# ablab/stringdecomposer

Measured on NVIDIA B200. Metric: dp_gcups, higher is better.
Workload: dtype s16x2

## Files before the change

stringdecomposer_b200/csrc/sweep_kernels.cu:

```cuda
#include <cuda_runtime.h>
#include <nvtx3/nvToolsExt.h>

#include <algorithm>
#include <climits>
#include <cstdio>
#include <cstdlib>
#include <cstring>
#include <mutex>
#include <string>
#include <vector>

#include "sweep_kernel.cuh"
#include "sweep_lat_kernel.cuh"
#include "filter_kernels.cuh"
#include "cuda_scope.h"
#include "block_cache.h"

namespace sdb {

#define SD_CUDA(x)                                                                                              \
    do {                                                                                                        \
        cudaError_t e_ = (x);                                                                                   \
        if (e_ != cudaSuccess) throw PlanError{std::string("CUDA error: ") + cudaGetErrorString(e_) + " at " +  \
                                               __FILE__ + ":" + std::to_string(__LINE__)};                      \
    } while (0)

struct TbArgs {
    Geometry g;
    const uint32_t *codes; const int64_t *cta_code_off;
    const JR *jr; const int64_t *seg_j_off;
    const uint8_t *bases; const int64_t *seg_off; int nseg;
    const uint8_t *rows; const int *row_off;
    int ins, del, mismatch, match;
    Record *scratch; const int64_t *seg_rec_off; int *counts;
    const int *rank2row;
    int *error;
    int invC;
};

constexpr int TB_WARPS = 4;
__global__ void __launch_bounds__(TB_WARPS * 32) traceback_kernel(const TbArgs a)
{
    const int s = blockIdx.x * TB_WARPS + (threadIdx.x >> 5);
    if (s >= a.nseg) return;
    const int lane = threadIdx.x & 31;
    const Geometry g = a.g;
    const int cta0 = g.NG > 1 ? s * g.NG : s / g.NS, seg_local = g.NG > 1 ? 0 : s % g.NS;
    const int64_t o = a.seg_off[s];
    const int n = (int)(a.seg_off[s + 1] - o);
    const uint8_t *seg = a.bases + o;
    const JR *jr = a.jr + a.seg_j_off[s];
    const size_t cstride = (size_t)g.NT * g.CW;
    const int C = g.C, CW = g.CW, cshift = g.packed ? 3 : 4, cpw = 1 << cshift, invC = a.invC;
    const int maxwl = g.T * CW - 1;
    Record *out = a.scratch + a.seg_rec_off[s];

    const int *r2r = a.rank2row ? a.rank2row + (size_t)s * (2 * g.M) : nullptr;
    auto row_of = [&](int kr) { return (unsigned)kr >= (unsigned)(2 * g.M) ? -1 : r2r ? r2r[kr] : kr; };
    int i = n - 1;
    int r = row_of(jr[n].row);
    if (r < 0) {
        if (lane == 0) { *a.error = 1; a.counts[s] = 0; }
        return;
    }
    int last = a.row_off[r + 1] - a.row_off[r] - 1;
    int k = last, end = i, end_score = jr[n].j, cnt = 0;
    constexpr int TB_RING = 8;
    __shared__ uint32_t s_ring[TB_WARPS][TB_RING][4][32];
    uint32_t (*ring)[4][32] = s_ring[threadIdx.x >> 5];
    int i0 = -1000, row0 = -1, half = 0, ni0 = -2000, cur = 0;
    uint32_t w0 = 0, w1 = 0, w2 = 0; int wb = 0; bool colok = false;
    const uint32_t *rowbase = nullptr;
    auto issue_window = [&](int slot, int iw, int kw) {
        const int c = iw - lane;
        const bool xok = c >= 0 && kw >= 1;
        int xb = 0;
        if (xok) {
            const int kp = max(kw - lane, 0);
            const int t = (kp * invC) >> 16;
            const int wl = t * CW + ((kp - t * C) >> cshift);
            xb = min(max(wl - 1, 0), max(maxwl - 2, 0));
            const uint32_t *col = rowbase + (size_t)c * cstride;
            const uint32_t d0 = (uint32_t)__cvta_generic_to_shared(&ring[slot][0][lane]);
            asm volatile("cp.async.ca.shared.global [%0], [%1], 4;" ::"r"(d0), "l"(col + xb) : "memory");
            asm volatile("cp.async.ca.shared.global [%0], [%1], 4;" ::"r"(d0 + 128u), "l"(col + min(xb + 1, maxwl)) : "memory");
            asm volatile("cp.async.ca.shared.global [%0], [%1], 4;" ::"r"(d0 + 256u), "l"(col + min(xb + 2, maxwl)) : "memory");
        }
        ring[slot][3][lane] = (uint32_t)xb | (xok ? 0x80000000u : 0u);
        asm volatile("cp.async.commit_group;" ::: "memory");
    };

    for (;;) {
        if (k == 0) {
            bool ins_move = false;
            if (i != 0) {
                const uint8_t m0 = a.rows[a.row_off[r]];
                const int s_here = m0 == seg[i] ? a.match : a.mismatch;
                const int s_prev = m0 == seg[i - 1] ? a.match : a.mismatch;
                const int h_here = jr[i].j + s_here;
                const int h_prev = (i == 1) ? s_prev : jr[i - 1].j + s_prev;
                ins_move = (h_here == h_prev + a.ins);
            }
            if (ins_move) { --i; continue; }
        } else {
            if (r != row0 || i > i0 || i <= i0 - 32) {
                if (r == row0 && i == ni0) {
                    i0 = ni0;
                    const int freed = cur;
                    cur = cur + 1 == TB_RING ? 0 : cur + 1;
                    issue_window(freed, i0 - 32 * (TB_RING - 1), k - 32 * (TB_RING - 1));
                } else {
                    i0 = i; row0 = r;
                    const RowPlace pl = place_row(g, seg_local, r);
                    half = pl.half;
                    rowbase = a.codes + a.cta_code_off[cta0 + (g.NG > 1 ? pl.grp : 0)] + (size_t)lane_tid(g.T, pl.ginst, 0) * CW;
                    asm volatile("cp.async.wait_all;" ::: "memory");
                    cur = 0;
#pragma unroll
                    for (int j = 0; j < TB_RING; ++j) issue_window(j, i - 32 * j, k - 32 * j);
                }
                ni0 = i0 - 32;
                asm volatile("cp.async.wait_group %0;" ::"n"(TB_RING - 1) : "memory");
                w0 = ring[cur][0][lane]; w1 = ring[cur][1][lane]; w2 = ring[cur][2][lane];
                const uint32_t meta = ring[cur][3][lane];
                wb = (int)(meta & 0x7fffffffu); colok = (meta >> 31) != 0;
            }
            const int dcur = i0 - i;
            const int kd = k - (lane - dcur);
            bool ok = colok && lane >= dcur && kd >= 1;
            int code = 2;
            {
                const int kq = max(kd, 0);
                const int t = (kq * invC) >> 16;
                const int kk = kq - t * C;
                const int wi = kk >> cshift;
                const int rel = t * CW + wi - wb;
                ok = ok && (unsigned)rel < 3u;
                const uint32_t w = rel == 0 ? w0 : rel == 1 ? w1 : w2;
                const int cc = kk & (cpw - 1);
                const int ncell = min(cpw, C - (wi << cshift));
                code = decode_code(w, g.packed, ncell, cc, half);
            }
            const bool stop = lane >= dcur && (!ok || code != 2);
            const unsigned ball = __ballot_sync(0xffffffffu, stop);
            const int f = ball ? __ffs(ball) - 1 : 32;
            const int steps = f - dcur;
            i -= steps; k -= steps;
            if (f == 32) continue;
            const int okf = __shfl_sync(0xffffffffu, (int)ok, f);
            const int codef = __shfl_sync(0xffffffffu, code, f);
            if (!okf) {
                if (k >= 1) row0 = -1;
                continue;
            }
            if (codef == 0) { --k; continue; }
            if (codef == 1) { --i; continue; }
        }
        if (cnt >= n) { cnt = -1; break; }
        Record rec;
        rec.row = r; rec.start = i; rec.end = end;
        if (i == 0) { rec.score = end_score; if (lane == 0) out[cnt] = rec; ++cnt; break; }
        const JR ji = jr[i];
        rec.score = end_score - ji.j;
        if (lane == 0) out[cnt] = rec;
        ++cnt;
        end_score = ji.j;
        r = row_of(ji.row);
        if (r < 0) {
            if (lane == 0) *a.error = 1;
            cnt = 0;
            break;
        }
        --i;
        last = a.row_off[r + 1] - a.row_off[r] - 1;
        k = last; end = i;
    }
    if (lane == 0) a.counts[s] = cnt;
}

__global__ void __launch_bounds__(1024) gather_kernel(const Record *scratch, const int64_t *seg_rec_off, const int *counts, Record *dense,
                                                      int nseg, int *total)
{
    __shared__ int s_warp[32];
    __shared__ int s_base, s_bad;
    const int tid = threadIdx.x, lane = tid & 31, warp = tid >> 5;
    if (tid == 0) { s_base = 0; s_bad = 0; }
    __syncthreads();
    for (int c0 = 0; c0 < nseg; c0 += 1024) {
        const int s = c0 + tid;
        const int c = s < nseg ? counts[s] : 0;
        if (c < 0) s_bad = 1;
        int v = c < 0 ? 0 : c;
#pragma unroll
        for (int d = 1; d < 32; d <<= 1) { const int o = __shfl_up_sync(0xffffffffu, v, d); if (lane >= d) v += o; }
        if (lane == 31) s_warp[warp] = v;
        __syncthreads();
        if (warp == 0) {
            int w = s_warp[lane];
#pragma unroll
            for (int d = 1; d < 32; d <<= 1) { const int o = __shfl_up_sync(0xffffffffu, w, d); if (lane >= d) w += o; }
            s_warp[lane] = w;
        }
        __syncthreads();
        const int start = s_base + (warp ? s_warp[warp - 1] : 0) + v - (c < 0 ? 0 : c);
        if (s < nseg && c > 0) {
            const Record *src = scratch + seg_rec_off[s];
            Record *dst = dense + start;
            for (int x = 0; x < c; ++x) dst[x] = src[c - 1 - x];
        }
        __syncthreads();
        if (tid == 0) s_base += s_warp[31];
        __syncthreads();
    }
    if (tid == 0) *total = s_bad ? -1 : s_base;
}

template <int MODE> __global__ void int_peak_kernel(unsigned *out, unsigned seed)
{
    unsigned r[8];
    const unsigned b = seed * 3u + threadIdx.x;
#pragma unroll
    for (int j = 0; j < 8; ++j) r[j] = threadIdx.x * 17u + j * 1315423911u + seed;
    for (int it = 0; it < 2048; ++it) {
#pragma unroll
        for (int j = 0; j < 8; ++j) {
            const unsigned nb = r[(j + 1) & 7];
            if (MODE == 0) r[j] = __viaddmax_s16x2(r[j], b, nb);
            else { r[j] = __viaddmax_s16x2(r[j], b, nb); r[j] = r[j] * b + nb; }
        }
    }
    unsigned acc = 0;
#pragma unroll
    for (int j = 0; j < 8; ++j) acc ^= r[j];
    out[blockIdx.x * blockDim.x + threadIdx.x] = acc;
}

static const void *sweep_kernel_for(const Geometry &g, bool fast, bool multi, bool timing)
{
    static const SweepLookup classic[2][3][2] = {
        {{sweep_lookup_s32_f0_m0, sweep_lookup_s32_f0_m0_st}, {sweep_lookup_s32_f1_m0, sweep_lookup_s32_f1_m0_st},
         {sweep_lookup_s32_f1_m1, sweep_lookup_s32_f1_m1_st}},
        {{sweep_lookup_p16_f0_m0, sweep_lookup_p16_f0_m0_st}, {sweep_lookup_p16_f1_m0, sweep_lookup_p16_f1_m0_st},
         {sweep_lookup_p16_f1_m1, sweep_lookup_p16_f1_m1_st}}};
    static const SweepLookup group[2] = {sweep_group_lookup_s32, sweep_group_lookup_p16};
    static const SweepLookup lat[2][2] = {{sweep_lat_lookup_s32, sweep_lat_lookup_s32_st}, {sweep_lat_lookup_p16, sweep_lat_lookup_p16_st}};
    const int pol = g.packed ? 1 : 0, st = g.stream ? 1 : 0;
    if (g.lat && timing) return pol && !st ? sweep_lat_timing_lookup_p16(g) : nullptr;
    if (g.lat) return lat[pol][st](g);
    if (g.NG > 1) return group[pol](g);
    return classic[pol][fast ? (multi ? 2 : 1) : 0][st](g);
}

namespace {

struct DevBuf {
    void *p = nullptr; size_t cap = 0; int dev = -1;
    void release()
    {
        if (!p) return;
// ... 57 lines not shown
constexpr size_t OUT_HDR = 16;
inline size_t out_counts_bytes(int nseg) { return ((size_t)nseg * 4 + 15) & ~size_t(15); }
inline int64_t wave_total(const int *hdr)
{
    if (hdr[1]) throw PlanError{"CUDA: sweep timed out waiting for a partner CTA (internal error)"};
    if (hdr[3]) throw PlanError{SD_MSG_TB_BAD_ROW};
    if (hdr[0]) throw PlanError{"segment contains a symbol outside ACGTN"};
    if (hdr[2] < 0) throw PlanError{"traceback overflowed its record buffer (internal error)"};
    return hdr[2];
}

struct WaveSlot {
    DevBuf d_bases, d_meta, d_codes, d_jr, d_scratch, d_out, d_dist, d_rank, d_r2r, d_segkj, d_xchg, d_dbg;
    MetaView d_segoff, d_ctanmax, d_ctacode, d_segj, d_segrec;
    PinnedBuf h_out;
    std::vector<char> hmeta;
    std::vector<int64_t> hoff;
    CtaLayout lay;
    int s0 = 0, s1 = 0, nseg = 0, nmax = 0;
    bool filter_on = false, staged = false;
    size_t nb = 0, rec_guess = 0;
    int end_idx = -1, prev_end = -1;
    cudaEvent_t ev[7]{};
};

class CudaBackend : public Backend {
public:
    explicit CudaBackend(int dev) : dev_(dev)
    {
        DeviceScope scope_(dev_); SD_CUDA(scope_.status);
        SD_CUDA(cudaStreamCreateWithFlags(&st_, cudaStreamNonBlocking));
        SD_CUDA(cudaStreamCreateWithFlags(&st_in_, cudaStreamNonBlocking));
        SD_CUDA(cudaStreamCreateWithFlags(&st_out_, cudaStreamNonBlocking));
        SD_CUDA(cudaStreamCreateWithFlags(&st_tb_, cudaStreamNonBlocking));
        SD_CUDA(cudaStreamCreateWithFlags(&st2_, cudaStreamNonBlocking));
        for (auto &w : slot_) for (auto &e : w.ev) SD_CUDA(cudaEventCreate(&e));
        for (auto &e : endev_) SD_CUDA(cudaEventCreate(&e));
        SD_CUDA(cudaGetDeviceProperties(&prop_, dev_));
        if (prop_.major != 10) throw PlanError{"CUDA device is not sm_100 class: this library carries sm_100a code only (no PTX for other architectures)"};
        size_t fr = 0, tot = 0;
        SD_CUDA(cudaMemGetInfo(&fr, &tot));
        free_at_start_ = (int64_t)fr;
        budget_ = std::min<int64_t>((int64_t)(fr * 0.85), (int64_t)96 << 30);
    }
    ~CudaBackend() override
    {
        DeviceScope scope_(dev_);
        cudaDeviceSynchronize();
        for (auto &w : slot_) for (auto &e : w.ev) cudaEventDestroy(e);
        for (auto &e : endev_) cudaEventDestroy(e);
        cudaStreamDestroy(st2_);
        cudaStreamDestroy(st_); cudaStreamDestroy(st_in_); cudaStreamDestroy(st_out_); cudaStreamDestroy(st_tb_);
    }
    const char *name() const override { return "cuda"; }

    void configure(const Plan &p, const MonomerSet &ms) override
    {
        DeviceScope scope_(dev_); SD_CUDA(scope_.status);
        plan_ = p; ms_ = ms;
        const Geometry &g = p.g;
        const int spw = 32 / g.T;
        fast_ = (g.nslots % spw == 0) && (g.nslots / spw <= 4) && g.NS <= 15;
        if (getenv("SD_NOFAST")) fast_ = false;
        lat_timing_ = g.lat && getenv("SD_LAT_TIMING") && sweep_kernel_for(g, fast_, false, true);
        kernel_ = sweep_kernel_for(g, fast_, fast_ && g.NS > 1, lat_timing_);
        if (g.lat && (g.NT / 32) * g.NG > 32) throw PlanError{"internal: a deferred-jump cluster holds at most 32 warps"};
        if (!kernel_) throw PlanError{"no sweep kernel compiled for this geometry"};
        cudaFuncAttributes fa;
        SD_CUDA(cudaFuncGetAttributes(&fa, kernel_));
        const int nthreads = g.NT * (g.NG > 1 && !g.lat ? g.NS : 1);
        if ((int64_t)((fa.numRegs + 7) / 8 * 8) * nthreads > 65536 || fa.maxThreadsPerBlock < nthreads)
            throw PlanError{"sweep geometry exceeds the register file (regs*threads > 64K)"};
        const std::vector<uint32_t> &table = g.lat ? p.prof2 : p.prof;
        d_prof_.need(table.size() * 4);
        SD_CUDA(cudaMemcpyAsync(d_prof_.p, table.data(), table.size() * 4, cudaMemcpyHostToDevice, st_));
        d_slotlen_.need(p.slot_len.size() * 4); d_slotend_.need(p.slot_endadd.size() * 4);
        SD_CUDA(cudaMemcpyAsync(d_slotlen_.p, p.slot_len.data(), p.slot_len.size() * 4, cudaMemcpyHostToDevice, st_));
        SD_CUDA(cudaMemcpyAsync(d_slotend_.p, p.slot_endadd.data(), p.slot_endadd.size() * 4, cudaMemcpyHostToDevice, st_));
        d_rows_.need(ms.rows.size()); d_rowoff_.need(ms.row_off.size() * 4);
        rows_ascii_.resize(ms.rows.size());
        for (size_t x = 0; x < ms.rows.size(); ++x) rows_ascii_[x] = (uint8_t)"ACGTN"[ms.rows[x]];
        SD_CUDA(cudaMemcpyAsync(d_rows_.p, rows_ascii_.data(), rows_ascii_.size(), cudaMemcpyHostToDevice, st_));
        SD_CUDA(cudaMemcpyAsync(d_rowoff_.p, ms.row_off.data(), ms.row_off.size() * 4, cudaMemcpyHostToDevice, st_));
        if (g.lat) {
            const int R = ms.nrows();
            kjbase_.assign((size_t)R * 5, 0);
            std::vector<int> one((size_t)R, -1);
            for (int r = 0; r < R; ++r) {
                one[(size_t)r] = 0;
                lat_jump_keys(ms, p.sc, one.data(), kjbase_.data() + (size_t)r * 5);
                one[(size_t)r] = -1;
            }
            d_kjbase_.need(kjbase_.size() * 4);
            SD_CUDA(cudaMemcpyAsync(d_kjbase_.p, kjbase_.data(), kjbase_.size() * 4, cudaMemcpyHostToDevice, st_));
        }
        SD_CUDA(cudaStreamSynchronize(st_));
    }

    int64_t wave_bytes(const Batch &b, int s0, int s1) const override
    {
        CtaLayout l = make_cta_layout(plan_, b, s0, s1);
        int64_t bytes = l.cta_code_off.back() * 4 + l.seg_j_off.back() * 8 + l.seg_rec_off.back() * 32 + (b.off[s1] - b.off[s0]);
        if (ed_thr_ >= 0) bytes += (int64_t)(s1 - s0) * ms_.nrows() * 12;
        return bytes;
    }
    int64_t wave_budget() const override
    {
        if (const char *e = getenv("SD_WAVE_BYTES")) if (atoll(e) > 0) return atoll(e);
        return budget_;
    }
    int64_t device_bytes() const override { return free_at_start_; }
    int wave_slots() const override { return 2; }

    void reserve(int slot, const Batch &b, int s0, int s1) override
    {
        DeviceScope scope_(dev_); SD_CUDA(scope_.status);
        WaveSlot &w = slot_[slot & 1];
        const CtaLayout lay = make_cta_layout(plan_, b, s0, s1);
        const int nseg = s1 - s0;
        w.d_bases.need((size_t)(b.off[s1] - b.off[s0]) + 16);
        w.d_codes.need((size_t)lay.cta_code_off.back() * 4 + 16);
        w.d_jr.need((size_t)lay.seg_j_off.back() * sizeof(JR) + 16);
        w.d_scratch.need((size_t)lay.seg_rec_off.back() * sizeof(Record) + 16);
        w.d_out.need(OUT_HDR + out_counts_bytes(nseg) + (size_t)lay.seg_rec_off.back() * sizeof(Record) + 64);
        w.h_out.need(OUT_HDR + out_counts_bytes(nseg) + ((size_t)(b.off[s1] - b.off[s0]) / 48 + (size_t)nseg * 4 + 64) * sizeof(Record));
    }

    void enqueue_h2d(WaveSlot &w, const Batch &b, int s0, int s1)
    {
        w.s0 = s0; w.s1 = s1; w.nseg = s1 - s0;
        w.lay = make_cta_layout(plan_, b, s0, s1);
        w.nmax = 0;
        for (int v : w.lay.cta_nmax) w.nmax = std::max(w.nmax, v);
        const int64_t base = b.off[s0];
        w.nb = (size_t)(b.off[s1] - base);
        w.hoff.resize((size_t)w.nseg + 1);
        for (int s = 0; s <= w.nseg; ++s) w.hoff[s] = b.off[s0 + s] - base;
        w.d_bases.need(w.nb + 16);
        const size_t msz[5] = {w.hoff.size() * 8, w.lay.cta_nmax.size() * 4, w.lay.cta_code_off.size() * 8, w.lay.seg_j_off.size() * 8,
                               w.lay.seg_rec_off.size() * 8};
        const void *msrc[5] = {w.hoff.data(), w.lay.cta_nmax.data(), w.lay.cta_code_off.data(), w.lay.seg_j_off.data(), w.lay.seg_rec_off.data()};
        MetaView *mdst[5] = {&w.d_segoff, &w.d_ctanmax, &w.d_ctacode, &w.d_segj, &w.d_segrec};
        size_t mtotal = 0, moff[5];
        for (int x = 0; x < 5; ++x) { moff[x] = mtotal; mtotal += (msz[x] + 255) & ~size_t(255); }
        w.d_meta.need(mtotal + 16);
        w.hmeta.resize(mtotal);
        for (int x = 0; x < 5; ++x) { memcpy(w.hmeta.data() + moff[x], msrc[x], msz[x]); mdst[x]->p = w.d_meta.as<char>() + moff[x]; }
        w.d_codes.need((size_t)w.lay.cta_code_off.back() * 4 + 16);
        w.d_jr.need((size_t)w.lay.seg_j_off.back() * sizeof(JR) + 16);
        w.d_scratch.need((size_t)w.lay.seg_rec_off.back() * sizeof(Record) + 16);
        w.rec_guess = (size_t)(w.nb / 48) + (size_t)w.nseg * 4 + 64;
        w.d_out.need(OUT_HDR + out_counts_bytes(w.nseg) + (size_t)w.lay.seg_rec_off.back() * sizeof(Record) + 64);
        SD_CUDA(cudaEventRecord(w.ev[0], st_in_));
        SD_CUDA(cudaMemcpyAsync(w.d_bases.p, b.text + base, w.nb, cudaMemcpyHostToDevice, st_in_));
        SD_CUDA(cudaMemcpyAsync(w.d_meta.p, w.hmeta.data(), mtotal, cudaMemcpyHostToDevice, st_in_));
        SD_CUDA(cudaMemsetAsync(w.d_out.p, 0, OUT_HDR, st_in_));
        SD_CUDA(cudaEventRecord(w.ev[1], st_in_));
        h2d_bytes += (int64_t)(w.nb + mtotal);
        w.filter_on = ed_thr_ >= 0;
        if (w.filter_on) build_filter(w);
        w.staged = true;
    }

    void build_filter(WaveSlot &w)
    {
        const int R = ms_.nrows();
        const size_t np = (size_t)w.nseg * R;
        w.d_dist.need(np * 4); w.d_rank.need(np * 4); w.d_r2r.need(np * 4);
        int *segkj = nullptr;
        if (plan_.g.lat) { w.d_segkj.need((size_t)w.nseg * 5 * 4); segkj = w.d_segkj.as<int>(); }
        SD_CUDA(launch_filter(w.d_bases.as<uint8_t>(), w.d_segoff.as<int64_t>(), w.nseg, w.nmax, d_rows_.as<uint8_t>(), d_rowoff_.as<int>(),
// ... 49 lines not shown
        a.error = w.d_out.as<int>() + 1;
        const int spw = 32 / g.T, wps = g.NT / 32;
        const size_t sgt = (size_t)wps * spw * g.T;
        const size_t smem = (size_t)5 * sgt * plan_.qp * 16 + ((size_t)g.NS * wps + g.NS + 8) * 4;
        if (smem > (size_t)prop_.sharedMemPerBlockOptin) throw PlanError{"group sweep needs more shared memory than the SM has"};
        SD_CUDA(cudaFuncSetAttribute(kernel_, cudaFuncAttributeMaxDynamicSharedMemorySize, (int)smem));
        int per_sm = 0;
        SD_CUDA(cudaOccupancyMaxActiveBlocksPerMultiprocessor(&per_sm, kernel_, g.NS * g.NT, smem));
        const int capacity = per_sm * prop_.multiProcessorCount;
        if (capacity < g.NG) throw PlanError{"monomer set too large: the CTAs of one segment cannot be co-resident on this GPU"};
        const int nblocks = (w.nseg + g.NS - 1) / g.NS;
        a.ngslots = std::min(nblocks, capacity / g.NG);
        if (const char *e = getenv("SD_GROUP_GSLOTS")) if (atoi(e) > 0) a.ngslots = std::min(a.ngslots, atoi(e));
        group_slots = std::max(group_slots, a.ngslots);
        const size_t xwords = (size_t)a.ngslots * 2 * g.NG * g.NS;
        w.d_xchg.need(xwords * 8);
        a.xbuf = w.d_xchg.as<unsigned long long>();
        SD_CUDA(cudaMemsetAsync(a.xbuf, 0, xwords * 8, st_));
        void *args[] = {(void *)&a};
        SD_CUDA(cudaLaunchCooperativeKernel(kernel_, dim3(a.ngslots * g.NG), dim3(g.NS * g.NT), args, smem, st_));
    }

    void launch_lat(WaveSlot &w, int seg_stride)
    {
        const Geometry &g = plan_.g;
        LatArgs a;
        fill_common_args(a, w);
        a.prof2 = d_prof_.as<uint4>(); a.nsl_total = plan_.nsl; a.qp2 = plan_.qp2;
        a.NG = g.NG; a.SG = g.SG;
        a.lat_th = plan_.lat_th; a.scanw = g.scanw;
        for (int q = 0; q < 5; ++q) a.kj[q] = plan_.kj[q];
        a.seg_kj = w.filter_on ? w.d_segkj.as<int>() : nullptr;
        a.seg_stride = seg_stride;
        a.error = w.d_out.as<int>() + 1;
        const int spw = 32 / g.T, wpc = g.NT / 32;
        a.dbg = nullptr;
        if (lat_timing_) { w.d_dbg.need((size_t)w.nseg * g.NG * wpc * 64); a.dbg = w.d_dbg.as<long long>(); SD_CUDA(cudaMemsetAsync(a.dbg, 0, (size_t)w.nseg * g.NG * wpc * 64, st_)); }
        const size_t sgt = (size_t)wpc * spw * g.T;
        const size_t smem = (size_t)5 * sgt * plan_.qp2 * 16 + (size_t)LAT_NBUF * 32 * 8 + 32 + (g.stream ? 0 : (size_t)seg_stride);
        if (smem > (size_t)prop_.sharedMemPerBlockOptin) throw PlanError{"deferred-jump sweep needs more shared memory than the SM has"};
        SD_CUDA(cudaFuncSetAttribute(kernel_, cudaFuncAttributeMaxDynamicSharedMemorySize, (int)smem));
        cudaLaunchConfig_t cfg{};
        cfg.gridDim = dim3((unsigned)(w.nseg * g.NG)); cfg.blockDim = dim3((unsigned)g.NT);
        cfg.dynamicSmemBytes = smem; cfg.stream = st_;
        cudaLaunchAttribute attr[1];
        attr[0].id = cudaLaunchAttributeClusterDimension;
        attr[0].val.clusterDim.x = (unsigned)g.NG; attr[0].val.clusterDim.y = 1; attr[0].val.clusterDim.z = 1;
        cfg.attrs = attr; cfg.numAttrs = 1;
        void *args[] = {(void *)&a};
        SD_CUDA(cudaLaunchKernelExC(&cfg, kernel_, args));
        if (lat_timing_) {
            const size_t nw = (size_t)w.nseg * g.NG * wpc;
            std::vector<long long> h(nw * 8);
            SD_CUDA(cudaMemcpyAsync(h.data(), a.dbg, nw * 64, cudaMemcpyDeviceToHost, st_));
            SD_CUDA(cudaStreamSynchronize(st_));
            double acc[6] = {0, 0, 0, 0, 0, 0}, cols = 0;
            for (size_t x = 0; x < nw; ++x) { for (int q = 0; q < 6; ++q) acc[q] += (double)h[x * 8 + q]; cols += (double)h[x * 8 + 6]; }
            fprintf(stderr, "[sd_b200 lat timing] cycles per column and warp: scan %.1f chain %.1f key+publish %.1f receive %.1f J+merge+store %.1f pre %.1f  (total %.1f)\n",
                    acc[0] / cols, acc[1] / cols, acc[2] / cols, acc[3] / cols, acc[4] / cols, acc[5] / cols,
                    (acc[0] + acc[1] + acc[2] + acc[3] + acc[4] + acc[5]) / cols);
        }
    }

    void enqueue_kernels(WaveSlot &w)
    {
        const Geometry &g = plan_.g;
        const int seg_stride = (w.nmax + 16) / 16 * 16;
        const bool own_stream = !g.lat && g.NG == 1 && &w == &slot_[1];
        cudaStream_t ss = own_stream ? st2_ : st_;
        SD_CUDA(cudaStreamWaitEvent(ss, w.ev[1], 0));
        SD_CUDA(cudaEventRecord(w.ev[2], ss));
        if (g.lat) launch_lat(w, seg_stride); else if (g.NG > 1) launch_group(w); else launch_single(w, seg_stride, ss);
        SD_CUDA(cudaEventRecord(w.ev[3], ss));
        w.prev_end = last_end_;
        w.end_idx = (int)(wave_seq_++ & 3);
        SD_CUDA(cudaEventRecord(endev_[w.end_idx], ss));
        last_end_ = w.end_idx;
        SD_CUDA(cudaStreamWaitEvent(st_tb_, w.ev[3], 0));
        SD_CUDA(cudaEventRecord(w.ev[6], st_tb_));
        TbArgs t;
        t.g = g; t.codes = w.d_codes.as<uint32_t>(); t.cta_code_off = w.d_ctacode.as<int64_t>(); t.jr = w.d_jr.as<JR>();
        t.seg_j_off = w.d_segj.as<int64_t>();
        t.bases = w.d_bases.as<uint8_t>(); t.seg_off = w.d_segoff.as<int64_t>(); t.nseg = w.nseg;
        t.rows = d_rows_.as<uint8_t>(); t.row_off = d_rowoff_.as<int>();
        t.ins = plan_.sc.ins; t.del = plan_.sc.del; t.mismatch = plan_.sc.mismatch; t.match = plan_.sc.match;
        t.scratch = w.d_scratch.as<Record>(); t.seg_rec_off = w.d_segrec.as<int64_t>();
        t.counts = reinterpret_cast<int *>(w.d_out.as<char>() + OUT_HDR);
        t.rank2row = w.filter_on ? w.d_r2r.as<int>() : nullptr;
        t.error = w.d_out.as<int>() + 3;
        t.invC = (65536 + g.C - 1) / g.C;
        for (int pos = 0; pos < g.C * g.T; ++pos)
            if (((pos * t.invC) >> 16) != pos / g.C) throw PlanError{"internal: reciprocal division inexact"};
        traceback_kernel<<<(w.nseg + TB_WARPS - 1) / TB_WARPS, TB_WARPS * 32, 0, st_tb_>>>(t);
        SD_CUDA(cudaGetLastError());
        SD_CUDA(cudaEventRecord(w.ev[4], st_tb_));
        launches += 2;
    }

    void enqueue_gather(WaveSlot &w)
    {
        char *ob = w.d_out.as<char>();
        Record *dense = reinterpret_cast<Record *>(ob + OUT_HDR + out_counts_bytes(w.nseg));
        gather_kernel<<<1, 1024, 0, st_tb_>>>(w.d_scratch.as<Record>(), w.d_segrec.as<int64_t>(), reinterpret_cast<int *>(ob + OUT_HDR),
                                          dense, w.nseg, reinterpret_cast<int *>(ob) + 2);
        SD_CUDA(cudaGetLastError());
        launches += 1;
    }

    void enqueue_d2h(WaveSlot &w)
    {
        const size_t first = OUT_HDR + out_counts_bytes(w.nseg) + w.rec_guess * sizeof(Record);
        const size_t cap = OUT_HDR + out_counts_bytes(w.nseg) + (size_t)w.lay.seg_rec_off.back() * sizeof(Record);
        w.h_out.need(std::min(first, cap));
        SD_CUDA(cudaEventRecord(w.ev[5], st_tb_));
        SD_CUDA(cudaStreamWaitEvent(st_out_, w.ev[5], 0));
        SD_CUDA(cudaMemcpyAsync(w.h_out.p, w.d_out.p, std::min(first, cap), cudaMemcpyDeviceToHost, st_out_));
        SD_CUDA(cudaEventRecord(w.ev[5], st_out_));
    }

    void finish(WaveSlot &w, BatchResult &out)
    {
        SD_CUDA(cudaEventSynchronize(w.ev[5]));
        const int64_t total = wave_total(w.h_out.as<int>());
        const size_t rec_off = OUT_HDR + out_counts_bytes(w.nseg);
        const size_t base = out.recs.size();
        out.recs.resize(base + (size_t)total);
        const size_t have = std::min<size_t>((size_t)total, w.rec_guess);
        if (have) memcpy(out.recs.data() + base, w.h_out.as<char>() + rec_off, have * sizeof(Record));
        if ((size_t)total > have) {
            SD_CUDA(cudaMemcpyAsync(out.recs.data() + base + have, w.d_out.as<char>() + rec_off + have * sizeof(Record),
                                    ((size_t)total - have) * sizeof(Record), cudaMemcpyDeviceToHost, st_out_));
            SD_CUDA(cudaStreamSynchronize(st_out_));
        }
        const int *cnt = reinterpret_cast<const int *>(w.h_out.as<char>() + OUT_HDR);
        int64_t run = (int64_t)base;
        for (int s = 0; s < w.nseg; ++s) { run += cnt[s]; out.rec_off.push_back(run); }
        float ms = 0;
        SD_CUDA(cudaEventElapsedTime(&ms, w.ev[0], w.ev[1])); h2d_ms += ms;
        SD_CUDA(cudaEventElapsedTime(&ms, w.ev[2], w.ev[3]));
        if (w.prev_end >= 0) {
            float since_prev = 0;
            SD_CUDA(cudaEventElapsedTime(&since_prev, endev_[w.prev_end], w.ev[3]));
            ms = std::min(ms, std::max(since_prev, 0.0f));
        }
        sweep_ms += ms;
        SD_CUDA(cudaEventElapsedTime(&ms, w.ev[6], w.ev[4])); traceback_ms += ms;
        d2h_bytes += (int64_t)(rec_off + (size_t)total * sizeof(Record));
        w.staged = false;
    }

    void submit(int slot, const Batch &b, int s0, int s1) override
    {
        DeviceScope scope_(dev_); SD_CUDA(scope_.status);
        WaveSlot &w = slot_[slot & 1];
        nvtxRangePushA("sd_b200: wave copy-in");
        enqueue_h2d(w, b, s0, s1);
        nvtxRangePop();
        nvtxRangePushA("sd_b200: wave sweep + traceback");
        enqueue_kernels(w);
        enqueue_gather(w);
        nvtxRangePop();
        nvtxRangePushA("sd_b200: wave copy-out");
        enqueue_d2h(w);
        nvtxRangePop();
    }
    void collect(int slot, BatchResult &out) override
    {
        DeviceScope scope_(dev_); SD_CUDA(scope_.status);
        nvtxRangePushA("sd_b200: wave collect");
        try { finish(slot_[slot & 1], out); } catch (...) { nvtxRangePop(); throw; }
        nvtxRangePop();
    }
    void stage(const Batch &b, int s0, int s1) override
    {
        DeviceScope scope_(dev_); SD_CUDA(scope_.status);
        enqueue_h2d(slot_[0], b, s0, s1);
        SD_CUDA(cudaStreamSynchronize(st_in_));
        float ms = 0; SD_CUDA(cudaEventElapsedTime(&ms, slot_[0].ev[0], slot_[0].ev[1])); h2d_ms += ms;
    }
    void execute() override
    {
        DeviceScope scope_(dev_); SD_CUDA(scope_.status);
        WaveSlot &w = slot_[0];
        SD_CUDA(cudaMemsetAsync(w.d_out.p, 0, OUT_HDR, st_));
        enqueue_kernels(w);
        int hdr[4] = {0, 0, 0, 0};
        SD_CUDA(cudaMemcpyAsync(hdr, w.d_out.p, OUT_HDR, cudaMemcpyDeviceToHost, st_tb_));
        SD_CUDA(cudaStreamSynchronize(st_tb_));
        wave_total(hdr);
        float ms = 0;
        SD_CUDA(cudaEventElapsedTime(&ms, w.ev[2], w.ev[3])); sweep_ms += ms;
        SD_CUDA(cudaEventElapsedTime(&ms, w.ev[6], w.ev[4])); traceback_ms += ms;
    }
    void fetch(BatchResult &out) override
    {
        DeviceScope scope_(dev_); SD_CUDA(scope_.status);
        WaveSlot &w = slot_[0];
        const double sw = sweep_ms, tb = traceback_ms, h2 = h2d_ms;
        enqueue_gather(w);
        enqueue_d2h(w);
        finish(w, out);
        sweep_ms = sw; traceback_ms = tb; h2d_ms = h2;
    }

private:
    int dev_;
    cudaStream_t st_{}, st_in_{}, st_out_{}, st_tb_{};
    cudaStream_t st2_{};
    cudaEvent_t endev_[4]{};
    uint64_t wave_seq_ = 0; int last_end_ = -1;
    cudaDeviceProp prop_{};
    Plan plan_; MonomerSet ms_;
    const void *kernel_ = nullptr;
    bool fast_ = false, lat_timing_ = false;
    std::vector<uint8_t> rows_ascii_;
    int64_t budget_ = 0;
    int64_t free_at_start_ = 0;
    DevBuf d_prof_, d_slotlen_, d_slotend_, d_rows_, d_rowoff_, d_kjbase_;
    std::vector<int> kjbase_;
    WaveSlot slot_[2];
};

}

Backend *make_cuda_backend(int device_id, std::string &err)
{
    try { return new CudaBackend(device_id); }
    catch (PlanError &e) { err = e.msg; return nullptr; }
}

}

int cuda_device_count()
{
    int n = 0;
    if (cudaGetDeviceCount(&n) != cudaSuccess) return 0;
    return n;
}

void *cuda_host_alloc(size_t bytes)
{
    void *p = nullptr;
    if (cudaHostAlloc(&p, bytes ? bytes : 1, cudaHostAllocPortable) != cudaSuccess) { cudaGetLastError(); return nullptr; }
    return p;
}

void cuda_host_free(void *p) { cudaFreeHost(p); }

int cuda_int_peak(int device, double *alu, double *both, double *mhz, std::string &err)
{
    using namespace sdb;
    try {
        DeviceScope scope_(device); SD_CUDA(scope_.status);
        cudaDeviceProp p; SD_CUDA(cudaGetDeviceProperties(&p, device));
        const int nblk = p.multiProcessorCount * 2, nthr = 512;
        unsigned *d; SD_CUDA(cudaMalloc(&d, (size_t)nblk * nthr * 4));
        cudaEvent_t e0, e1; SD_CUDA(cudaEventCreate(&e0)); SD_CUDA(cudaEventCreate(&e1));
        double res[2] = {0, 0};
        for (int mode = 0; mode < 2; ++mode) {
            float best = 1e30f;
            for (int rep = 0; rep < 5; ++rep) {
                SD_CUDA(cudaEventRecord(e0));
                if (mode == 0) int_peak_kernel<0><<<nblk, nthr>>>(d, 1234u); else int_peak_kernel<1><<<nblk, nthr>>>(d, 1234u);
                SD_CUDA(cudaEventRecord(e1));
                SD_CUDA(cudaEventSynchronize(e1));
                float ms; SD_CUDA(cudaEventElapsedTime(&ms, e0, e1));
                if (rep > 0) best = std::min(best, ms);
            }
            const double ops = (double)nblk * nthr * 2048.0 * 8.0 * (mode == 0 ? 1.0 : 2.0);
            res[mode] = ops / (best * 1e-3);
        }
        if (alu) *alu = res[0];
        if (both) *both = res[1];
        if (mhz) *mhz = res[0] / ((double)p.multiProcessorCount * 64.0) / 1e6;
        cudaEventDestroy(e0); cudaEventDestroy(e1); cudaFree(d);
    } catch (PlanError &e) { err = e.msg; return 4; }
    return 0;
}
```

Baseline: 2740.

## Prefetch next row's traceback windows and nearby JR/base data into double-buffered shared ring

The traceback kernel now precomputes a per-slot row table (last column, code word offset, group, first symbol, half) on the host, which replaces the place_row, row_off and cta_code_off lookups done inside the kernel. At each row transition it predicts the next row from the JR entry and issues cp.async prefetches of that row's code windows, plus a window of nearby JR records and sequence bytes, into a second shared-memory buffer. Boundary and insertion checks read JR and bases from shared memory through warp shuffles instead of global loads. This aims to hide the global-load latency of the serial traceback chain, at the cost of doubling shared memory per warp and adding more complex wait-group bookkeeping. The codes base now uses cta_code_off[cta0] plus grp*n*cstride, which assumes a particular layout when NG>1.

New measurement: 2697, median of 6. 1.6% lower.

```diff
diff --git a/stringdecomposer_b200/csrc/sweep_kernels.cu b/stringdecomposer_b200/csrc/sweep_kernels.cu
--- a/stringdecomposer_b200/csrc/sweep_kernels.cu
+++ b/stringdecomposer_b200/csrc/sweep_kernels.cu
@@ -25,12 +25,20 @@
                                                __FILE__ + ":" + std::to_string(__LINE__)};                      \
     } while (0)
 
+struct alignas(16) TbRow {
+    int32_t last;
+    int32_t word;
+    int32_t grp;
+    uint8_t sym, half;
+    uint8_t pad_[2];
+};
+
 struct TbArgs {
     Geometry g;
     const uint32_t *codes; const int64_t *cta_code_off;
     const JR *jr; const int64_t *seg_j_off;
     const uint8_t *bases; const int64_t *seg_off; int nseg;
-    const uint8_t *rows; const int *row_off;
+    const TbRow *rowtab;
     int ins, del, mismatch, match;
     Record *scratch; const int64_t *seg_rec_off; int *counts;
     const int *rank2row;
@@ -39,9 +47,13 @@
 };
 
 constexpr int TB_WARPS = 4;
+constexpr int TB_RING = 8;
+constexpr int TB_NEAR = 32;
+constexpr int TB_AIM = 8;
 __global__ void __launch_bounds__(TB_WARPS * 32) traceback_kernel(const TbArgs a)
 {
-    const int s = blockIdx.x * TB_WARPS + (threadIdx.x >> 5);
+    const int wid = threadIdx.x >> 5;
+    const int s = blockIdx.x * TB_WARPS + wid;
     if (s >= a.nseg) return;
     const int lane = threadIdx.x & 31;
     const Geometry g = a.g;
@@ -54,6 +66,13 @@
     const int C = g.C, CW = g.CW, cshift = g.packed ? 3 : 4, cpw = 1 << cshift, invC = a.invC;
     const int maxwl = g.T * CW - 1;
     Record *out = a.scratch + a.seg_rec_off[s];
+    const uint32_t *codes = a.codes + a.cta_code_off[cta0];
+    const TbRow *rowtab = a.rowtab + (size_t)seg_local * (2 * g.M);
+    struct RowInfo { int last, sym, half; const uint32_t *base; };
+    auto row_info = [&](int r) {
+        const uint4 v = __ldg(reinterpret_cast<const uint4 *>(rowtab + r));
+        return RowInfo{(int)v.x, (int)(v.w & 0xffu), (int)((v.w >> 8) & 0xffu), codes + (size_t)v.z * n * cstride + v.y};
+    };
 
     const int *r2r = a.rank2row ? a.rank2row + (size_t)s * (2 * g.M) : nullptr;
     auto row_of = [&](int kr) { return (unsigned)kr >= (unsigned)(2 * g.M) ? -1 : r2r ? r2r[kr] : kr; };
@@ -63,15 +82,18 @@
         if (lane == 0) { *a.error = 1; a.counts[s] = 0; }
         return;
     }
-    int last = a.row_off[r + 1] - a.row_off[r] - 1;
-    int k = last, end = i, end_score = jr[n].j, cnt = 0;
-    constexpr int TB_RING = 8;
-    __shared__ uint32_t s_ring[TB_WARPS][TB_RING][4][32];
-    uint32_t (*ring)[4][32] = s_ring[threadIdx.x >> 5];
-    int i0 = -1000, row0 = -1, half = 0, ni0 = -2000, cur = 0;
+    RowInfo ri = row_info(r);
+    int k = ri.last, end = i, end_score = jr[n].j, cnt = 0;
+    __shared__ uint32_t s_ring[TB_WARPS][2][TB_RING][4][32];
+    __shared__ uint2 s_njr[TB_WARPS][2][TB_NEAR];
+    __shared__ uint32_t s_nsym[TB_WARPS][2][TB_NEAR];
+    int rb = 0, nb = 0;
+    int i0 = -1000, row0 = -1, ni0 = -2000, cur = 0;
     uint32_t w0 = 0, w1 = 0, w2 = 0; int wb = 0; bool colok = false;
-    const uint32_t *rowbase = nullptr;
-    auto issue_window = [&](int slot, int iw, int kw) {
+    int nlo = INT_MIN / 2, nal = 0;
+    int nx_row = -1, nx_i0 = 0, nx_lo = 0, nx_al = 0; RowInfo nx_ri{0, 0, 0, nullptr};
+    int older = 0;
+    auto issue_window = [&](int ringi, const uint32_t *rowbase, int slot, int iw, int kw) {
         const int c = iw - lane;
         const bool xok = c >= 0 && kw >= 1;
         int xb = 0;
@@ -81,49 +103,97 @@
             const int wl = t * CW + ((kp - t * C) >> cshift);
             xb = min(max(wl - 1, 0), max(maxwl - 2, 0));
             const uint32_t *col = rowbase + (size_t)c * cstride;
-            const uint32_t d0 = (uint32_t)__cvta_generic_to_shared(&ring[slot][0][lane]);
+            const uint32_t d0 = (uint32_t)__cvta_generic_to_shared(&s_ring[wid][ringi][slot][0][lane]);
             asm volatile("cp.async.ca.shared.global [%0], [%1], 4;" ::"r"(d0), "l"(col + xb) : "memory");
             asm volatile("cp.async.ca.shared.global [%0], [%1], 4;" ::"r"(d0 + 128u), "l"(col + min(xb + 1, maxwl)) : "memory");
             asm volatile("cp.async.ca.shared.global [%0], [%1], 4;" ::"r"(d0 + 256u), "l"(col + min(xb + 2, maxwl)) : "memory");
         }
-        ring[slot][3][lane] = (uint32_t)xb | (xok ? 0x80000000u : 0u);
+        s_ring[wid][ringi][slot][3][lane] = (uint32_t)xb | (xok ? 0x80000000u : 0u);
         asm volatile("cp.async.commit_group;" ::: "memory");
+    };
+    auto issue_near = [&](int b, int c, int &al) {
+        const int lo = max(0, min(c - TB_NEAR / 2, n + 1 - TB_NEAR));
+        if (lo + lane <= n) {
+            const uint32_t d = (uint32_t)__cvta_generic_to_shared(&s_njr[wid][b][lane]);
+            asm volatile("cp.async.ca.shared.global [%0], [%1], 8;" ::"r"(d), "l"(jr + lo + lane) : "memory");
+        }
+        al = (int)((uintptr_t)(seg + lo) & 3u);
+        const uint8_t *wsrc = seg + lo - al + 4 * lane;
+        if (lane < (TB_NEAR + 3) / 4 + 1 && wsrc < seg + n) {
+            const uint32_t d = (uint32_t)__cvta_generic_to_shared(&s_nsym[wid][b][lane]);
+            asm volatile("cp.async.ca.shared.global [%0], [%1], 4;" ::"r"(d), "l"(wsrc) : "memory");
+        }
+        asm volatile("cp.async.commit_group;" ::: "memory");
+        return lo;
+    };
+    auto close_data = [&](int c, JR &jc, int &jprev, int &sc, int &sprev) {
+        if (c - 1 >= nlo && c < nlo + TB_NEAR) {
+            const uint2 mj = s_njr[wid][nb][lane];
+            const uint32_t ms = s_nsym[wid][nb][lane];
+            jc.j = (int)__shfl_sync(0xffffffffu, mj.x, c - nlo); jc.row = (int)__shfl_sync(0xffffffffu, mj.y, c - nlo);
+            jprev = (int)__shfl_sync(0xffffffffu, mj.x, c - 1 - nlo);
+            const int q = c - nlo + nal;
+            sc = (int)((__shfl_sync(0xffffffffu, ms, q >> 2) >> (8 * (q & 3))) & 0xffu);
+            sprev = (int)((__shfl_sync(0xffffffffu, ms, (q - 1) >> 2) >> (8 * ((q - 1) & 3))) & 0xffu);
+        } else {
+            jc = jr[c]; jprev = jr[c - 1].j; sc = seg[c]; sprev = seg[c - 1];
+        }
+    };
+    auto issue_next = [&]() {
+        const int c = i - k;
+        if (c < 1 || c < nlo || c >= nlo + TB_NEAR) return;
+        const int kr = (int)__shfl_sync(0xffffffffu, s_njr[wid][nb][lane].y, c - nlo);
+        const int nr = row_of(kr);
+        if (nr < 0) return;
+        nx_ri = row_info(nr);
+        const int aim = min(TB_AIM, n - c);
+        nx_row = nr; nx_i0 = c - 1 + aim;
+        nx_lo = issue_near(nb ^ 1, c - 1 - nx_ri.last, nx_al);
+#pragma unroll
+        for (int j = 0; j < TB_RING; ++j) issue_window(rb ^ 1, nx_ri.base, j, nx_i0 - 32 * j, nx_ri.last + aim - 32 * j);
+        older = TB_RING - 1;
     };
 
     for (;;) {
         if (k == 0) {
             bool ins_move = false;
             if (i != 0) {
-                const uint8_t m0 = a.rows[a.row_off[r]];
-                const int s_here = m0 == seg[i] ? a.match : a.mismatch;
-                const int s_prev = m0 == seg[i - 1] ? a.match : a.mismatch;
-                const int h_here = jr[i].j + s_here;
-                const int h_prev = (i == 1) ? s_prev : jr[i - 1].j + s_prev;
+                JR jh; int jp, sh, sp;
+                close_data(i, jh, jp, sh, sp);
+                const int s_here = ri.sym == sh ? a.match : a.mismatch;
+                const int s_prev = ri.sym == sp ? a.match : a.mismatch;
+                const int h_here = jh.j + s_here;
+                const int h_prev = (i == 1) ? s_prev : jp + s_prev;
                 ins_move = (h_here == h_prev + a.ins);
             }
             if (ins_move) { --i; continue; }
         } else {
             if (r != row0 || i > i0 || i <= i0 - 32) {
-                if (r == row0 && i == ni0) {
+                bool fresh = true;
+                if (r == nx_row && i <= nx_i0 && i > nx_i0 - 32) {
+                    asm volatile("cp.async.wait_all;" ::: "memory");
+                    rb ^= 1; nb ^= 1; nlo = nx_lo; nal = nx_al;
+                    i0 = nx_i0; row0 = r; cur = 0; older = 0;
+                } else if (r == row0 && i == ni0) {
                     i0 = ni0;
                     const int freed = cur;
                     cur = cur + 1 == TB_RING ? 0 : cur + 1;
-                    issue_window(freed, i0 - 32 * (TB_RING - 1), k - 32 * (TB_RING - 1));
+                    issue_window(rb, ri.base, freed, i0 - 32 * (TB_RING - 1), k - 32 * (TB_RING - 1));
+                    fresh = false;
                 } else {
-                    i0 = i; row0 = r;
-                    const RowPlace pl = place_row(g, seg_local, r);
-                    half = pl.half;
-                    rowbase = a.codes + a.cta_code_off[cta0 + (g.NG > 1 ? pl.grp : 0)] + (size_t)lane_tid(g.T, pl.ginst, 0) * CW;
                     asm volatile("cp.async.wait_all;" ::: "memory");
-                    cur = 0;
+                    i0 = i; row0 = r; cur = 0; older = 0;
+                    nlo = issue_near(nb, i - k, nal);
 #pragma unroll
-                    for (int j = 0; j < TB_RING; ++j) issue_window(j, i - 32 * j, k - 32 * j);
+                    for (int j = 0; j < TB_RING; ++j) issue_window(rb, ri.base, j, i - 32 * j, k - 32 * j);
                 }
                 ni0 = i0 - 32;
-                asm volatile("cp.async.wait_group %0;" ::"n"(TB_RING - 1) : "memory");
-                w0 = ring[cur][0][lane]; w1 = ring[cur][1][lane]; w2 = ring[cur][2][lane];
-                const uint32_t meta = ring[cur][3][lane];
+                if (older > 0) { --older; asm volatile("cp.async.wait_group %0;" ::"n"(TB_RING - 1 + TB_RING + 1) : "memory"); }
+                else asm volatile("cp.async.wait_group %0;" ::"n"(TB_RING - 1) : "memory");
+                w0 = s_ring[wid][rb][cur][0][lane]; w1 = s_ring[wid][rb][cur][1][lane]; w2 = s_ring[wid][rb][cur][2][lane];
+                const uint32_t meta = s_ring[wid][rb][cur][3][lane];
                 wb = (int)(meta & 0x7fffffffu); colok = (meta >> 31) != 0;
+                if (fresh) { nx_row = -1; issue_next(); }
             }
             const int dcur = i0 - i;
             const int kd = k - (lane - dcur);
@@ -139,7 +209,7 @@
                 const uint32_t w = rel == 0 ? w0 : rel == 1 ? w1 : w2;
                 const int cc = kk & (cpw - 1);
                 const int ncell = min(cpw, C - (wi << cshift));
-                code = decode_code(w, g.packed, ncell, cc, half);
+                code = decode_code(w, g.packed, ncell, cc, ri.half);
             }
             const bool stop = lane >= dcur && (!ok || code != 2);
             const unsigned ball = __ballot_sync(0xffffffffu, stop);
@@ -150,7 +220,7 @@
             const int okf = __shfl_sync(0xffffffffu, (int)ok, f);
             const int codef = __shfl_sync(0xffffffffu, code, f);
             if (!okf) {
-                if (k >= 1) row0 = -1;
+                if (k >= 1) { row0 = -1; nx_row = -1; }
                 continue;
             }
             if (codef == 0) { --k; continue; }
@@ -160,7 +230,8 @@
         Record rec;
         rec.row = r; rec.start = i; rec.end = end;
         if (i == 0) { rec.score = end_score; if (lane == 0) out[cnt] = rec; ++cnt; break; }
-        const JR ji = jr[i];
+        JR ji; int jp_, sh_, sp_;
+        close_data(i, ji, jp_, sh_, sp_);
         rec.score = end_score - ji.j;
         if (lane == 0) out[cnt] = rec;
         ++cnt;
@@ -172,8 +243,8 @@
             break;
         }
         --i;
-        last = a.row_off[r + 1] - a.row_off[r] - 1;
-        k = last; end = i;
+        ri = r == nx_row ? nx_ri : row_info(r);
+        k = ri.last; end = i;
     }
     if (lane == 0) a.counts[s] = cnt;
 }
@@ -398,11 +469,22 @@
         for (size_t x = 0; x < ms.rows.size(); ++x) rows_ascii_[x] = (uint8_t)"ACGTN"[ms.rows[x]];
         SD_CUDA(cudaMemcpyAsync(d_rows_.p, rows_ascii_.data(), rows_ascii_.size(), cudaMemcpyHostToDevice, st_));
         SD_CUDA(cudaMemcpyAsync(d_rowoff_.p, ms.row_off.data(), ms.row_off.size() * 4, cudaMemcpyHostToDevice, st_));
+        const int npos = g.NG > 1 ? 1 : g.NS, nrows = ms.nrows();
+        tbrow_.assign((size_t)npos * nrows, TbRow{});
+        for (int sl = 0; sl < npos; ++sl)
+            for (int r = 0; r < nrows; ++r) {
+                const RowPlace pl = place_row(g, sl, r);
+                TbRow &e = tbrow_[(size_t)sl * nrows + r];
+                e.last = ms.rowlen(r) - 1; e.word = lane_tid(g.T, pl.ginst, 0) * g.CW; e.grp = pl.grp;
+                e.sym = rows_ascii_[(size_t)ms.row_off[r]]; e.half = (uint8_t)pl.half;
+            }
+        d_tbrow_.need(tbrow_.size() * sizeof(TbRow));
+        SD_CUDA(cudaMemcpyAsync(d_tbrow_.p, tbrow_.data(), tbrow_.size() * sizeof(TbRow), cudaMemcpyHostToDevice, st_));
         if (g.lat) {
             const int R = ms.nrows();
             kjbase_.assign((size_t)R * 5, 0);
             std::vector<int> one((size_t)R, -1);
-            for (int r = 0; r < R; ++r) {
+            for (int r = 0; r < nrows; ++r) {
                 one[(size_t)r] = 0;
                 lat_jump_keys(ms, p.sc, one.data(), kjbase_.data() + (size_t)r * 5);
                 one[(size_t)r] = -1;
@@ -618,7 +700,7 @@
         t.g = g; t.codes = w.d_codes.as<uint32_t>(); t.cta_code_off = w.d_ctacode.as<int64_t>(); t.jr = w.d_jr.as<JR>();
         t.seg_j_off = w.d_segj.as<int64_t>();
         t.bases = w.d_bases.as<uint8_t>(); t.seg_off = w.d_segoff.as<int64_t>(); t.nseg = w.nseg;
-        t.rows = d_rows_.as<uint8_t>(); t.row_off = d_rowoff_.as<int>();
+        t.rowtab = d_tbrow_.as<TbRow>();
         t.ins = plan_.sc.ins; t.del = plan_.sc.del; t.mismatch = plan_.sc.mismatch; t.match = plan_.sc.match;
         t.scratch = w.d_scratch.as<Record>(); t.seg_rec_off = w.d_segrec.as<int64_t>();
         t.counts = reinterpret_cast<int *>(w.d_out.as<char>() + OUT_HDR);
@@ -750,9 +832,10 @@
     const void *kernel_ = nullptr;
     bool fast_ = false, lat_timing_ = false;
     std::vector<uint8_t> rows_ascii_;
+    std::vector<TbRow> tbrow_;
     int64_t budget_ = 0;
     int64_t free_at_start_ = 0;
-    DevBuf d_prof_, d_slotlen_, d_slotend_, d_rows_, d_rowoff_, d_kjbase_;
+    DevBuf d_prof_, d_slotlen_, d_slotend_, d_rows_, d_rowoff_, d_kjbase_, d_tbrow_;
     std::vector<int> kjbase_;
     WaveSlot slot_[2];
 };
```

## Prefetch next row's traceback window speculatively and cache row tables in shared memory

Applied to the files above, without the earlier changes.

The traceback kernel now uses a double-buffered per-warp cp.async ring. Each slot also prefetches the JR entries and sequence bytes for the window's columns. When a row jump is predicted, the ring for the next row is fetched speculatively, and a hit swaps buffers without a fresh cold fetch. Row offsets, first symbols and the per-segment rank2row map are staged into dynamic shared memory, which cuts scattered global loads at a cost in smem footprint, occupancy, extra wait_all points and code complexity.

Result: slower. 2738 before, 2697 after, median of 6 (-1.5%).

```diff
diff --git a/stringdecomposer_b200/csrc/sweep_kernels.cu b/stringdecomposer_b200/csrc/sweep_kernels.cu
--- a/stringdecomposer_b200/csrc/sweep_kernels.cu
+++ b/stringdecomposer_b200/csrc/sweep_kernels.cu
@@ -39,12 +39,35 @@
 };
 
 constexpr int TB_WARPS = 4;
+constexpr int TB_RING = 8;
+constexpr int TB_SLOT_WORDS = 7 * 32;
+constexpr int TB_W_META = 3 * 32, TB_W_JR = 4 * 32, TB_W_SYM = 6 * 32;
+inline size_t tb_smem_bytes(int nrows, bool filter)
+{
+    return (size_t)TB_WARPS * 2 * TB_RING * TB_SLOT_WORDS * 4 + (size_t)(nrows + 1) * 4 +
+           (filter ? (size_t)TB_WARPS * nrows * 4 : 0) + (size_t)nrows;
+}
+
 __global__ void __launch_bounds__(TB_WARPS * 32) traceback_kernel(const TbArgs a)
 {
+    extern __shared__ __align__(16) uint32_t tb_smem[];
+    const Geometry g = a.g;
+    const int nrows = 2 * g.M;
+    int *const s_roff = reinterpret_cast<int *>(tb_smem + TB_WARPS * 2 * TB_RING * TB_SLOT_WORDS);
+    int *const s_r2r = s_roff + nrows + 1;
+    uint8_t *const s_first = reinterpret_cast<uint8_t *>(s_r2r + (a.rank2row ? TB_WARPS * nrows : 0));
+    for (int x = threadIdx.x; x <= nrows; x += blockDim.x) s_roff[x] = a.row_off[x];
+    for (int x = threadIdx.x; x < nrows; x += blockDim.x) s_first[x] = a.rows[a.row_off[x]];
     const int s = blockIdx.x * TB_WARPS + (threadIdx.x >> 5);
+    const int lane = threadIdx.x & 31;
+    const int *r2r = nullptr;
+    if (a.rank2row && s < a.nseg) {
+        int *mine = s_r2r + (threadIdx.x >> 5) * nrows;
+        for (int x = lane; x < nrows; x += 32) mine[x] = a.rank2row[(size_t)s * nrows + x];
+        r2r = mine;
+    }
+    __syncthreads();
     if (s >= a.nseg) return;
-    const int lane = threadIdx.x & 31;
-    const Geometry g = a.g;
     const int cta0 = g.NG > 1 ? s * g.NG : s / g.NS, seg_local = g.NG > 1 ? 0 : s % g.NS;
     const int64_t o = a.seg_off[s];
     const int n = (int)(a.seg_off[s + 1] - o);
@@ -53,52 +76,115 @@
     const size_t cstride = (size_t)g.NT * g.CW;
     const int C = g.C, CW = g.CW, cshift = g.packed ? 3 : 4, cpw = 1 << cshift, invC = a.invC;
     const int maxwl = g.T * CW - 1;
+    const int64_t code0 = g.NG > 1 ? 0 : a.cta_code_off[cta0];
     Record *out = a.scratch + a.seg_rec_off[s];
 
-    const int *r2r = a.rank2row ? a.rank2row + (size_t)s * (2 * g.M) : nullptr;
-    auto row_of = [&](int kr) { return (unsigned)kr >= (unsigned)(2 * g.M) ? -1 : r2r ? r2r[kr] : kr; };
+    auto row_of = [&](int kr) { return (unsigned)kr >= (unsigned)nrows ? -1 : r2r ? r2r[kr] : kr; };
+    auto row_last = [&](int row) { return s_roff[row + 1] - s_roff[row] - 1; };
+    auto row_base = [&](int row, int &hf) {
+        const RowPlace pl = place_row(g, seg_local, row);
+        hf = pl.half;
+        return a.codes + (g.NG > 1 ? a.cta_code_off[cta0 + pl.grp] : code0) + (size_t)lane_tid(g.T, pl.ginst, 0) * CW;
+    };
     int i = n - 1;
     int r = row_of(jr[n].row);
     if (r < 0) {
         if (lane == 0) { *a.error = 1; a.counts[s] = 0; }
         return;
     }
-    int last = a.row_off[r + 1] - a.row_off[r] - 1;
+    int last = row_last(r);
     int k = last, end = i, end_score = jr[n].j, cnt = 0;
-    constexpr int TB_RING = 8;
-    __shared__ uint32_t s_ring[TB_WARPS][TB_RING][4][32];
-    uint32_t (*ring)[4][32] = s_ring[threadIdx.x >> 5];
+    uint32_t *const rings = tb_smem + (threadIdx.x >> 5) * 2 * TB_RING * TB_SLOT_WORDS;
+    auto slot_at = [&](int ring, int slot) { return rings + (ring * TB_RING + slot) * TB_SLOT_WORDS; };
+    int rb = 0;
     int i0 = -1000, row0 = -1, half = 0, ni0 = -2000, cur = 0;
+    int ncomp = 0;
     uint32_t w0 = 0, w1 = 0, w2 = 0; int wb = 0; bool colok = false;
     const uint32_t *rowbase = nullptr;
-    auto issue_window = [&](int slot, int iw, int kw) {
+    auto fetch_window = [&](uint32_t *slot, int iw, int kw, const uint32_t *rbase) {
         const int c = iw - lane;
         const bool xok = c >= 0 && kw >= 1;
         int xb = 0;
+        const uint32_t d0 = (uint32_t)__cvta_generic_to_shared(slot + lane);
         if (xok) {
             const int kp = max(kw - lane, 0);
             const int t = (kp * invC) >> 16;
             const int wl = t * CW + ((kp - t * C) >> cshift);
             xb = min(max(wl - 1, 0), max(maxwl - 2, 0));
-            const uint32_t *col = rowbase + (size_t)c * cstride;
-            const uint32_t d0 = (uint32_t)__cvta_generic_to_shared(&ring[slot][0][lane]);
+            const uint32_t *col = rbase + (size_t)c * cstride;
             asm volatile("cp.async.ca.shared.global [%0], [%1], 4;" ::"r"(d0), "l"(col + xb) : "memory");
             asm volatile("cp.async.ca.shared.global [%0], [%1], 4;" ::"r"(d0 + 128u), "l"(col + min(xb + 1, maxwl)) : "memory");
             asm volatile("cp.async.ca.shared.global [%0], [%1], 4;" ::"r"(d0 + 256u), "l"(col + min(xb + 2, maxwl)) : "memory");
         }
-        ring[slot][3][lane] = (uint32_t)xb | (xok ? 0x80000000u : 0u);
-        asm volatile("cp.async.commit_group;" ::: "memory");
+        if (c >= 0) {
+            const uint32_t dj = (uint32_t)__cvta_generic_to_shared(slot + TB_W_JR + 2 * lane);
+            asm volatile("cp.async.ca.shared.global [%0], [%1], 8;" ::"r"(dj), "l"(jr + c) : "memory");
+            const uint8_t *sw = reinterpret_cast<const uint8_t *>(reinterpret_cast<uintptr_t>(seg + c) & ~uintptr_t(3));
+            asm volatile("cp.async.ca.shared.global [%0], [%1], 4;" ::"r"(d0 + 4u * TB_W_SYM), "l"(sw) : "memory");
+        }
+        slot[TB_W_META + lane] = (uint32_t)xb | (xok ? 0x80000000u : 0u);
+    };
+    auto commit = [] { asm volatile("cp.async.commit_group;" ::: "memory"); };
+    auto wait_all = [] { asm volatile("cp.async.wait_all;" ::: "memory"); };
+
+    bool sp_live = false;
+    bool sp_pend = false;
+    int sp_col = -1, sp_kr = -1, sp_r = -1, sp_half = 0, post = 0;
+    const uint32_t *sp_base = nullptr;
+
+    auto col_at = [&](int c, int &jj, int &jrow, int &sym) {
+        const int d = i0 - c;
+        if (c >= 0 && d >= 0 && d < 32 * TB_RING) {
+            if (d >= 32 * ncomp) { wait_all(); ncomp = TB_RING; sp_pend = false; }
+            int sl = cur + (d >> 5); if (sl >= TB_RING) sl -= TB_RING;
+            const uint32_t *e = slot_at(rb, sl);
+            const int own = i0 - (d & ~31) - lane;
+            const uint32_t sw = own >= 0 ? e[TB_W_SYM + lane] >> ((reinterpret_cast<uintptr_t>(seg + own) & 3) * 8) : 0u;
+            const int src = d & 31;
+            jj = __shfl_sync(0xffffffffu, (int)e[TB_W_JR + 2 * lane], src);
+            jrow = __shfl_sync(0xffffffffu, (int)e[TB_W_JR + 2 * lane + 1], src);
+            sym = __shfl_sync(0xffffffffu, (int)(sw & 0xffu), src);
+        } else {
+            const JR v = jr[c];
+            jj = v.j; jrow = v.row; sym = seg[c];
+        }
+    };
+    auto load_head = [&] {
+        const uint32_t *e = slot_at(rb, cur);
+        w0 = e[lane]; w1 = e[32 + lane]; w2 = e[64 + lane];
+        const uint32_t meta = e[TB_W_META + lane];
+        wb = (int)(meta & 0x7fffffffu); colok = (meta >> 31) != 0;
+    };
+    auto try_spec = [&] {
+        if (sp_live || k < 1) return;
+        const int p = i - k, d = i0 - p;
+        if (p < 1 || d < 0 || d >= 32 * ncomp) return;
+        int sl = cur + (d >> 5); if (sl >= TB_RING) sl -= TB_RING;
+        const int kr = __shfl_sync(0xffffffffu, (int)slot_at(rb, sl)[TB_W_JR + 2 * lane + 1], d & 31);
+        const int r2 = row_of(kr);
+        if (r2 < 0) return;
+        if (sp_pend) { wait_all(); sp_pend = false; }
+        sp_base = row_base(r2, sp_half);
+        const int k2 = row_last(r2);
+#pragma unroll
+        for (int j = 0; j < TB_RING; ++j) fetch_window(slot_at(1 - rb, j), p - 1 - 32 * j, k2 - 32 * j, sp_base);
+        commit();
+        sp_live = true; sp_pend = true; post = 0;
+        sp_col = p; sp_kr = kr; sp_r = r2;
     };
 
     for (;;) {
         if (k == 0) {
             bool ins_move = false;
             if (i != 0) {
-                const uint8_t m0 = a.rows[a.row_off[r]];
-                const int s_here = m0 == seg[i] ? a.match : a.mismatch;
-                const int s_prev = m0 == seg[i - 1] ? a.match : a.mismatch;
-                const int h_here = jr[i].j + s_here;
-                const int h_prev = (i == 1) ? s_prev : jr[i - 1].j + s_prev;
+                const int m0 = s_first[r];
+                int j_here, j_prev, row_x, c_here, c_prev;
+                col_at(i, j_here, row_x, c_here);
+                col_at(i - 1, j_prev, row_x, c_prev);
+                const int s_here = m0 == c_here ? a.match : a.mismatch;
+                const int s_prev = m0 == c_prev ? a.match : a.mismatch;
+                const int h_here = j_here + s_here;
+                const int h_prev = (i == 1) ? s_prev : j_prev + s_prev;
                 ins_move = (h_here == h_prev + a.ins);
             }
             if (ins_move) { --i; continue; }
@@ -108,22 +194,28 @@
                     i0 = ni0;
                     const int freed = cur;
                     cur = cur + 1 == TB_RING ? 0 : cur + 1;
-                    issue_window(freed, i0 - 32 * (TB_RING - 1), k - 32 * (TB_RING - 1));
+                    fetch_window(slot_at(rb, freed), i0 - 32 * (TB_RING - 1), k - 32 * (TB_RING - 1), rowbase);
+                    commit();
+                    if (sp_pend) ++post;
+                    if (ncomp < 2) {
+                        if (sp_pend && post <= TB_RING - 1) asm volatile("cp.async.wait_group %0;" ::"n"(TB_RING) : "memory");
+                        else asm volatile("cp.async.wait_group %0;" ::"n"(TB_RING - 1) : "memory");
+                    }
+                    ncomp = max(ncomp - 1, 1);
                 } else {
                     i0 = i; row0 = r;
-                    const RowPlace pl = place_row(g, seg_local, r);
-                    half = pl.half;
-                    rowbase = a.codes + a.cta_code_off[cta0 + (g.NG > 1 ? pl.grp : 0)] + (size_t)lane_tid(g.T, pl.ginst, 0) * CW;
-                    asm volatile("cp.async.wait_all;" ::: "memory");
+                    rowbase = row_base(r, half);
+                    wait_all();
                     cur = 0;
 #pragma unroll
-                    for (int j = 0; j < TB_RING; ++j) issue_window(j, i - 32 * j, k - 32 * j);
+                    for (int j = 0; j < TB_RING; ++j) fetch_window(slot_at(rb, j), i - 32 * j, k - 32 * j, rowbase);
+                    commit();
+                    wait_all();
+                    ncomp = TB_RING; sp_pend = false;
                 }
                 ni0 = i0 - 32;
-                asm volatile("cp.async.wait_group %0;" ::"n"(TB_RING - 1) : "memory");
-                w0 = ring[cur][0][lane]; w1 = ring[cur][1][lane]; w2 = ring[cur][2][lane];
-                const uint32_t meta = ring[cur][3][lane];
-                wb = (int)(meta & 0x7fffffffu); colok = (meta >> 31) != 0;
+                load_head();
+                try_spec();
             }
             const int dcur = i0 - i;
             const int kd = k - (lane - dcur);
@@ -160,21 +252,33 @@
         Record rec;
         rec.row = r; rec.start = i; rec.end = end;
         if (i == 0) { rec.score = end_score; if (lane == 0) out[cnt] = rec; ++cnt; break; }
-        const JR ji = jr[i];
-        rec.score = end_score - ji.j;
+        int ji, jrow, sym_x;
+        col_at(i, ji, jrow, sym_x);
+        rec.score = end_score - ji;
         if (lane == 0) out[cnt] = rec;
         ++cnt;
-        end_score = ji.j;
-        r = row_of(ji.row);
+        end_score = ji;
+        const bool hit = sp_live && sp_col == i && sp_kr == jrow;
+        r = hit ? sp_r : row_of(jrow);
         if (r < 0) {
             if (lane == 0) *a.error = 1;
             cnt = 0;
             break;
         }
         --i;
-        last = a.row_off[r + 1] - a.row_off[r] - 1;
+        last = row_last(r);
         k = last; end = i;
-    }
+        if (hit) {
+            wait_all();
+            rb = 1 - rb;
+            i0 = i; row0 = r; half = sp_half; rowbase = sp_base;
+            cur = 0; ni0 = i0 - 32; ncomp = TB_RING; sp_pend = false;
+            load_head();
+        }
+        sp_live = false;
+        if (hit) try_spec();
+    }
+    wait_all();
     if (lane == 0) a.counts[s] = cnt;
 }
 
@@ -627,7 +731,13 @@
         t.invC = (65536 + g.C - 1) / g.C;
         for (int pos = 0; pos < g.C * g.T; ++pos)
             if (((pos * t.invC) >> 16) != pos / g.C) throw PlanError{"internal: reciprocal division inexact"};
-        traceback_kernel<<<(w.nseg + TB_WARPS - 1) / TB_WARPS, TB_WARPS * 32, 0, st_tb_>>>(t);
+        const size_t tb_smem = tb_smem_bytes(ms_.nrows(), w.filter_on);
+        if (tb_smem > (size_t)prop_.sharedMemPerBlockOptin) throw PlanError{"traceback needs more shared memory than the SM has"};
+        if ((int)tb_smem > tb_smem_attr_) {
+            SD_CUDA(cudaFuncSetAttribute(traceback_kernel, cudaFuncAttributeMaxDynamicSharedMemorySize, (int)tb_smem));
+            tb_smem_attr_ = (int)tb_smem;
+        }
+        traceback_kernel<<<(w.nseg + TB_WARPS - 1) / TB_WARPS, TB_WARPS * 32, tb_smem, st_tb_>>>(t);
         SD_CUDA(cudaGetLastError());
         SD_CUDA(cudaEventRecord(w.ev[4], st_tb_));
         launches += 2;
@@ -749,6 +859,7 @@
     Plan plan_; MonomerSet ms_;
     const void *kernel_ = nullptr;
     bool fast_ = false, lat_timing_ = false;
+    int tb_smem_attr_ = 0;
     std::vector<uint8_t> rows_ascii_;
     int64_t budget_ = 0;
     int64_t free_at_start_ = 0;
```
